# mkofler96/DeepSDF

Measured on AMD Instinct MI355X. Metric: SDF point-samples/sec per training step (8x512 decoder, 16384 pts), higher is better.
Workload: dtype f32; 1 GPU; configs[1]: 64 synthetic sphere-SDF scenes, latent_dim=256, 8x512 decoder + layer-4 skip, weight-norm, dropout 0.2, 16384 pts/step (64 scenes x 256 samples), fp32; headline_config=True, parallelism=dp1

## Files before the change

deepsdf_amd/csrc/dsdf_api.hip:

```cpp
#include "../../include/dsdf.h"

#include <hip/hip_runtime.h>
#include <math.h>
#include <stdarg.h>
#include <stdio.h>
#include <string.h>

#include <stdlib.h>

#include <algorithm>
#include <atomic>
#ifdef DSDF_LAB
#include <vector>
#endif

#include "dwstream.hpp"
#include "sample.hpp"
#include "fused.hpp"
#include "fused_bf16x8.hpp"
#include "gemm.hpp"
#include "kernels.hpp"
#include "mcubes.hpp"
#include "meshsdf.hpp"
#include "msgrid.hpp"
// ... 1052 lines not shown
  R.dw_busy = want_dw ? ((R.dw_items + 3) / 4 < R.cus ? (R.dw_items + 3) / 4 : R.cus) : 0;
  static const bool no_ride = [] { const char* e = getenv("DSDF_NO_RIDE"); return e && e[0] == '1'; }();
  R.rides = segmode && want_dw && R.cus - R.dw_busy >= 8 && c.P.nwg <= R.cus && !no_ride && !c.net->gemm_split && phase <= 1 &&
            R.dw_items > 0;
  if (R.rides) {
    q.lat.nslice = 1; R.lat_slices = 1;
    q.lat_bx = 0;
    R.lat_n = (c.net->latent_size + 15) / 16;
    q.rr_n = q.rr_bx;
    q.dw_n = (q.dw.out[0] + SDW_ROWS_RIDE - 1) / SDW_ROWS_RIDE + (ks > 0 ? (q.dw.out[1] + SDW_ROWS_RIDE - 1) / SDW_ROWS_RIDE : 0);
  }
  return R;
}

int launch_dw(const Call& c, const DwSched& DS, const Roles& R, bool segmode, int phase) {
  const int last = c.net->n_layers - 1;
  DwArgs d;
  memset(&d, 0, sizeof(d));
  d.n_layers = last; d.n_full = DS.n_full; d.n_narrow = DS.n_narrow; d.N = (int)c.n;
  double fl = 0;
  for (int l = 0; l < last; ++l) {
    DwLayer& y = d.ly[l];
    y.dp = c.at<float>(c.P.dpl_off[l]); y.ld_dp = c.P.ld_dp;
    y.act = c.at<float>(c.P.in_off[l]); y.ld_act = c.P.ld_in[l];
    y.slabs = c.at<float>(c.P.dwslab_off[l]); y.slab = DS.slab[l];
    y.M = c.net->out_dim[l]; y.Nc = dw_cols(c.net, l, segmode); y.ldc = c.P.ld_in[l];
    y.tiles_m = DS.tiles_m[l]; y.tiles_n = DS.tiles_n[l]; y.last_nj = DS.last_nj[l]; y.nfull_n = DS.nfull_n[l];
    y.nsplit = DS.nsplit[l]; y.kchunk = DS.kchunk[l]; y.full0 = DS.full0[l]; y.narrow0 = DS.narrow0[l];
    if (in_phase(c.P, phase, l)) fl += 2.0 * (double)c.n * y.M * c.net->in_dim[l];
  }
#ifdef DSDF_LAB
  static LabStamps stamps{"DSDF_LAB_DWDBG", 1024 * 4 * 8 * 8, true, nullptr};
  LabScope lab(stamps, c.st);
  d.dbg = stamps.dev;
#endif
  ProfScope ps(DSDF_PROF_DW_STREAM, fl, c.st);
  const DwKernel kernel = KERNELS[c.path.family].dw;
  if (R.rides) {
    hipLaunchKernelGGL(kernel, dim3(R.cus), dim3(256), 0, c.st, d, R.q, R.lat_n, R.dw_busy);
  } else {
    PostBwdArgs none;
    memset(&none, 0, sizeof(none));
    const int grid = R.dw_busy < 1 ? 1 : R.dw_busy;
    hipLaunchKernelGGL(kernel, dim3(grid), dim3(256), 0, c.st, d, none, 0, grid);
  }
  LAUNCH_OK("dw_stream_kernel");
  return 0;
}

int fin_table(const Call& c, const DwSched& DS, const GradSink& to, bool segmode, int phase, FinAll* fa) {
  const int last = c.net->n_layers - 1, ks = skip_layer(c.net);
  memset(fa, 0, sizeof(*fa));
  int rows = 0;
  for (int l = last; l >= 0; --l) {
    if (!in_phase(c.P, phase, l)) continue;
    FinSrc src;
    if (l == last) src = FinSrc{c.at<float>(c.P.part2_off), LAST_GROUPS, c.P.ld_part, c.P.ld_part, c.at<float>(c.P.partdb_off), c.P.nwg, 1};
    else if (l == last - 1)
      src = FinSrc{c.at<float>(c.P.dwslab_off[l]), DS.nsplit[l], DS.slab[l], c.P.ld_in[l], c.at<float>(c.P.part2_off) + c.P.ld_in[last], LAST_GROUPS, c.P.ld_part};
    else src = FinSrc{c.at<float>(c.P.dwslab_off[l]), DS.nsplit[l], DS.slab[l], c.P.ld_in[l], c.at<float>(c.P.cs_off[l]), c.P.nwg, c.P.ldcs};
    FinArgs& f = fa->f[fa->n];
    f = fin_args(c, l, src, to);
    if (segmode && (l == 0 || l == ks)) {
      f.hoist = 1; f.lat0 = l == 0 ? 0 : c.net->out_dim[l - 1]; f.hW = c.net->latent_size + c.net->geom_dim; f.ldh = c.P.ldh;
      f.hs = c.at<float>(c.P.hs_off) + (l == 0 ? 0 : c.P.hstride);
    }
    fa->row0[fa->n] = rows;
    rows += fin_blocks(f.out, f.in);
    ++fa->n;
  }
  fa->row0[fa->n] = rows;
  return rows;
}

int run_backward_fused(const Call& c, const GradSink& to, int ncols_dz, bool* used_dzB, bool want_dw, const FusedBwdHead& head,
                       const SegBwd* sb, const FusedFwdArgs* fwd, int phase) {
  const DwSched& DS = phase == 0 ? c.P.dw : c.P.dwph[phase - 1];
  const bool segmode = sb != nullptr;
  FusedBwdArgs a = dx_chain_args(c, ncols_dz, want_dw, head, sb, used_dzB);
  if (phase <= 1) TRY(launch_dx_chain(c, a, fwd));
  const Roles R = plan_roles(c, DS, want_dw, sb, phase);
  if (!segmode && phase <= 1 && want_dw) {
    hipLaunchKernelGGL(reduce_rows_kernel, dim3(R.rr_bx, LAST_GROUPS), dim3(256), 0, c.st, R.rr);
    LAUNCH_OK("reduce_rows_kernel");
  }
  if (segmode && sb->scatter != nullptr) { sb->scatter->nslice = R.lat_slices; sb->scatter->slice_stride = (long long)sb->R * c.net->latent_size; }
  if (segmode && !R.rides && phase <= 1) {
    hipLaunchKernelGGL(post_bwd_kernel, dim3((unsigned)(R.q.rr_n + R.q.dw_n + R.lat_n)), dim3(256), 0, c.st, R.q, R.lat_n);
    LAUNCH_OK("post_bwd_kernel");
  }
  if (!want_dw) return 0;
  if (R.dw_items > 0) TRY(launch_dw(c, DS, R, segmode, phase));
  FinAll fa;
  const int rows = fin_table(c, DS, to, segmode, phase, &fa);
  if (rows == 0) return 0;
  if (segmode && sb->scatter != nullptr && phase <= 1) {
    hipLaunchKernelGGL(finalize_scatter_kernel, dim3(rows + sb->R), dim3(256), 0, c.st, fa, *sb->scatter, rows);
    LAUNCH_OK("finalize_scatter_kernel");
    *sb->scatter_done = true;
  } else {
    hipLaunchKernelGGL(finalize_all_kernel, dim3(rows), dim3(256), 0, c.st, fa);
    LAUNCH_OK("finalize_all_kernel");
  }
  return 0;
}

FusedBwdHead make_head(const Call& c, int mode) {
  const int last = c.net->n_layers - 1;
  FusedBwdHead h;
  memset(&h, 0, sizeof(h));
  h.mode = mode;
  h.a_last = c.at<float>(c.P.in_off[last]); h.ld_a = c.P.ld_in[last]; h.in_last = c.net->in_dim[last];
  h.w_last = c.packed + c.pk.w_off[last]; h.b_last = c.params + c.L.bias_off[last]; h.use_tanh = c.net->use_tanh;
// ... 1867 lines not shown
```

deepsdf_amd/csrc/dwstream.hpp:

```cpp
#pragma once
#include "common.hpp"
#include "fused.hpp"
#include "kernels.hpp"

namespace dsdf {

struct DwLayer {
  const float* dp; int ld_dp;
  const float* act; int ld_act;
  float* slabs; long long slab;
  int M, Nc, ldc;
  int tiles_m, tiles_n;
  int last_nj;
  int nfull_n;
  int nsplit, kchunk;
  int full0, narrow0;
};
struct DwArgs { int n_layers, n_full, n_narrow, N; DwLayer ly[DSDF_MAX_LAYERS];
                unsigned long long* dbg; };

#ifndef DW_RING_STEPS
#define DW_RING_STEPS 16
#endif
constexpr int DW_RING = DW_RING_STEPS;

template <int NJ> struct DwVec;
template <> struct DwVec<1> { typedef float type; };
template <> struct DwVec<2> { typedef float2 type; };
template <> struct DwVec<3> { typedef float3 type; };
template <> struct DwVec<4> { typedef float4 type; };

template <int NJ>
__device__ __forceinline__ void dw_item(const DwLayer& L, int N, int split, int m0, int n0, int kbeg, int kend, int fr, int fh) {
  typedef typename DwVec<NJ>::type bvec;
  const int nsteps = (kend - kbeg) >> 1;
  const float* bq = L.act + (size_t)(kbeg + fh) * L.ld_act + n0 + NJ * fr;
  const size_t bstep = (size_t)2 * L.ld_act;
  typedef uint32_t u32x4 __attribute__((ext_vector_type(4)));
  const size_t rows_left = (size_t)(N - kbeg);
  const int ra_bytes = (int)min(rows_left * L.ld_dp * 4, (size_t)0x7FFFFFFF), rb_bytes = (int)min(rows_left * L.ld_act * 4, (size_t)0x7FFFFFFF);
  const __amdgpu_buffer_rsrc_t ra = __builtin_amdgcn_make_buffer_rsrc((void*)(L.dp + (size_t)kbeg * L.ld_dp), 0, ra_bytes, 0x00020000);
  const __amdgpu_buffer_rsrc_t rb = __builtin_amdgcn_make_buffer_rsrc((void*)(L.act + (size_t)kbeg * L.ld_act), 0, rb_bytes, 0x00020000);
  const int voa = (fh * L.ld_dp + m0 + 4 * fr) * 4, vob = (fh * L.ld_act + n0 + NJ * fr) * 4;
  const int astepb = 8 * L.ld_dp, bstepb = 8 * L.ld_act;
  auto lda = [&](int q) -> float4 {
    const u32x4 r = __builtin_amdgcn_raw_buffer_load_b128(ra, voa, q * astepb, 0);
    return make_float4(__uint_as_float(r.x), __uint_as_float(r.y), __uint_as_float(r.z), __uint_as_float(r.w));
  };

  f32x16 acc[4][NJ];
#pragma unroll
  for (int i = 0; i < 4; ++i)
#pragma unroll
    for (int j = 0; j < NJ; ++j)
#pragma unroll
      for (int r = 0; r < 16; ++r) acc[i][j][r] = 0.f;

  float4 rga[DW_RING];
  bvec rgb[DW_RING];
  auto ldb = [&](const float* q) -> bvec {
    if constexpr (NJ == 3) { bvec v; v.x = q[0]; v.y = q[1]; v.z = q[2]; return v; }
    else return *reinterpret_cast<const bvec*>(q);
  };
  auto ldbq = [&](int q) -> bvec {
    if constexpr (NJ == 4) {
      const u32x4 r = __builtin_amdgcn_raw_buffer_load_b128(rb, vob, q * bstepb, 0);
      return make_float4(__uint_as_float(r.x), __uint_as_float(r.y), __uint_as_float(r.z), __uint_as_float(r.w));
    } else return ldb(bq + (size_t)q * bstep);
  };
  auto mma = [&](const float4& a, const bvec& b) {
    const float av[4] = {a.x, a.y, a.z, a.w};
    float bv[NJ];
    if constexpr (NJ == 1) bv[0] = b;
    else { bv[0] = b.x; bv[1] = b.y; if constexpr (NJ > 2) bv[2] = b.z; if constexpr (NJ > 3) bv[3] = b.w; }
#pragma unroll
    for (int i = 0; i < 4; ++i)
#pragma unroll
      for (int j = 0; j < NJ; ++j) acc[i][j] = __builtin_amdgcn_mfma_f32_32x32x2f32(av[i], bv[j], acc[i][j], 0, 0, 0);
  };
  if (nsteps > 0) {
    const int last = nsteps - 1;
#pragma unroll
    for (int q = 0; q < DW_RING - 1; ++q) {
      rga[q] = lda(min(q, last));
      rgb[q] = ldbq(min(q, last));
    }
    int s = 0;
    for (; s + DW_RING <= nsteps; s += DW_RING) {
#pragma unroll
      for (int q = 0; q < DW_RING; ++q) {
        const int nxt = min(s + q + DW_RING - 1, last);
        rga[(q + DW_RING - 1) % DW_RING] = lda(nxt);
        rgb[(q + DW_RING - 1) % DW_RING] = ldbq(nxt);
        mma(rga[q], rgb[q]);
        if constexpr (NJ == 4) {
          __builtin_amdgcn_sched_group_barrier(0x020, 1, 0);
          __builtin_amdgcn_sched_group_barrier(0x008, 8, 0);
          __builtin_amdgcn_sched_group_barrier(0x020, 1, 0);
          __builtin_amdgcn_sched_group_barrier(0x008, 8, 0);
        }
      }
    }
#pragma unroll
    for (int q = 0; q < DW_RING - 1; ++q)
      if (s + q < nsteps) mma(rga[q], rgb[q]);
  }
  if ((kend - kbeg) & 1) {
    const int k = kend - 1;
    float4 a = make_float4(0.f, 0.f, 0.f, 0.f);
    bvec b;
    if constexpr (NJ == 1) b = 0.f; else { b.x = 0.f; b.y = 0.f; if constexpr (NJ > 2) b.z = 0.f; if constexpr (NJ > 3) b.w = 0.f; }
    if (fh == 0) {
      a = *reinterpret_cast<const float4*>(L.dp + (size_t)k * L.ld_dp + m0 + 4 * fr);
      b = ldb(L.act + (size_t)k * L.ld_act + n0 + NJ * fr);
    }
    mma(a, b);
  }

  float* slab = L.slabs + (size_t)split * L.slab;
  __amdgpu_buffer_rsrc_t rs = __builtin_amdgcn_make_buffer_rsrc((void*)slab, 0, L.M * L.ldc * 4, 0x00020000);
  const int n = n0 + NJ * fr;
#pragma unroll
  for (int i = 0; i < 4; ++i)
#pragma unroll
    for (int r = 0; r < 16; ++r) {
      const int m = m0 + 4 * (crow(r) + 4 * fh) + i;
      if constexpr (NJ == 4) {
        typedef uint32_t u32x4 __attribute__((ext_vector_type(4)));
        const uint32_t voff = n < L.ldc ? (uint32_t)((m * L.ldc + n) * 4) : 0x7FFFFFFFu;
        u32x4 v = {__float_as_uint(acc[i][0][r]), __float_as_uint(acc[i][1][r]), __float_as_uint(acc[i][2][r]),
                   __float_as_uint(acc[i][3][r])};
        __builtin_amdgcn_raw_buffer_store_b128(v, rs, voff, 0, 0);
      } else {
#pragma unroll
        for (int j = 0; j < NJ; ++j) {
          const uint32_t voff = n + j < L.ldc ? (uint32_t)((m * L.ldc + n + j) * 4) : 0x7FFFFFFFu;
          __builtin_amdgcn_raw_buffer_store_b32(__float_as_uint(acc[i][j][r]), rs, voff, 0, 0);
        }
      }
    }
}

constexpr int DWS_RING = 4;
constexpr int DWS_SLOT = 2 * 16 * 256;

__device__ __forceinline__ Split3 split8v(const float (&x)[8]) {
  typedef uint32_t u32x4 __attribute__((ext_vector_type(4)));
  uint32_t hw[4], mw[4], lw[4];
#pragma unroll
  for (int pr = 0; pr < 4; ++pr) cut_pair(x[2 * pr], x[2 * pr + 1], hw[pr], mw[pr], lw[pr]);
  Split3 s;
  s.h = __builtin_bit_cast(bf16x8, (u32x4){hw[0], hw[1], hw[2], hw[3]});
  s.m = __builtin_bit_cast(bf16x8, (u32x4){mw[0], mw[1], mw[2], mw[3]});
  s.l = __builtin_bit_cast(bf16x8, (u32x4){lw[0], lw[1], lw[2], lw[3]});
  return s;
}

typedef float dw_f32x4 __attribute__((ext_vector_type(4)));
template <int J> __device__ __forceinline__ float dw_comp(const dw_f32x4& v) { return J == 0 ? v.x : (J == 1 ? v.y : (J == 2 ? v.z : v.w)); }
struct DwRaw { dw_f32x4 v[8]; };

__device__ __forceinline__ void dw_block_split(const DwLayer& L, int split, int tmb, int tnb, int kbeg, int kend, int w, int lane, float* ring) {
  typedef uint32_t u32x4 __attribute__((ext_vector_type(4)));
  typedef __attribute__((address_space(3))) void* lds_ptr;
  typedef __attribute__((address_space(3))) const float* lds_cf;
  const int fr = lane & 31, fh = lane >> 5;
  const int npts = kend - kbeg, nsteps = (npts + 15) >> 4;
  const __amdgpu_buffer_rsrc_t ra = __builtin_amdgcn_make_buffer_rsrc((void*)(L.dp + (size_t)kbeg * L.ld_dp), 0, npts * L.ld_dp * 4, 0x00020000);
  const __amdgpu_buffer_rsrc_t rb = __builtin_amdgcn_make_buffer_rsrc((void*)(L.act + (size_t)kbeg * L.ld_act), 0, npts * L.ld_act * 4, 0x00020000);
  const int pva = (tmb * 128 + 4 * lane) * 4, pvb = (tnb * 128 + 4 * lane) * 4;
  auto issue = [&](int st) __attribute__((always_inline)) {
    float* slot = ring + (st % DWS_RING) * DWS_SLOT;
#pragma unroll
    for (int rr = 0; rr < 4; ++rr) {
      const int row = 4 * w + rr, pt = 16 * st + row;
      __builtin_amdgcn_raw_ptr_buffer_load_lds(ra, (lds_ptr)(slot + row * 256), 16, pt * L.ld_dp * 4 + pva, 0, 0, 0);
      __builtin_amdgcn_raw_ptr_buffer_load_lds(rb, (lds_ptr)(slot + 4096 + row * 256), 16, pt * L.ld_act * 4 + pvb, 0, 0, 0);
    }
  };
  int lda4 = L.ld_dp * 4, ldb4 = L.ld_act * 4;
  asm volatile("" : "+s"(lda4), "+s"(ldb4));
  auto issue_row = [&](int st, int rr) __attribute__((always_inline)) {
    float* slot = ring + (st % DWS_RING) * DWS_SLOT;
    int row = 4 * w + rr;
    asm volatile("" : "+s"(row));
    const int pt = 16 * st + row;
    __builtin_amdgcn_raw_ptr_buffer_load_lds(ra, (lds_ptr)(slot + row * 256), 16, pt * lda4 + pva, 0, 0, 0);
    __builtin_amdgcn_raw_ptr_buffer_load_lds(rb, (lds_ptr)(slot + 4096 + row * 256), 16, pt * ldb4 + pvb, 0, 0, 0);
  };
  const int ca = (w >> 1) * 128 + 4 * fr, cb = 4096 + (w & 1) * 128 + 4 * fr;
#define DW_READ_RAW(ST, A, B, WAITSTR)                                                                                              \
  {                                                                                                                                 \
    const float* slot_ = ring + ((ST) % DWS_RING) * DWS_SLOT;                                                                       \
// ... 123 lines not shown
#undef DW_SBSEL
#undef DW_SA_OF
#undef DW_WAIT_LGKM
#undef DW_READ_RAW
  __builtin_amdgcn_s_waitcnt(0x0F70);
  __syncthreads();
  const int m0 = (tmb + (w >> 1)) * 128, n0 = (tnb + (w & 1)) * 128;
  float* slab = L.slabs + (size_t)split * L.slab;
  __amdgpu_buffer_rsrc_t rs = __builtin_amdgcn_make_buffer_rsrc((void*)slab, 0, L.M * L.ldc * 4, 0x00020000);
  const int n = n0 + 4 * fr;
#pragma unroll
  for (int i = 0; i < 4; ++i)
#pragma unroll
    for (int rg = 0; rg < 16; ++rg) {
      const int m = m0 + 4 * (crow(rg) + 4 * fh) + i;
      const uint32_t voff = n < L.ldc ? (uint32_t)((m * L.ldc + n) * 4) : 0x7FFFFFFFu;
      u32x4 v = {__float_as_uint(acc[i][0][rg]), __float_as_uint(acc[i][1][rg]), __float_as_uint(acc[i][2][rg]),
                 __float_as_uint(acc[i][3][rg])};
      __builtin_amdgcn_raw_buffer_store_b128(v, rs, voff, 0, 0);
    }
}

template <bool SPLIT>
__device__ __forceinline__ void dw_stream_body(const DwArgs& p, const PostBwdArgs& post, const int post_lat_n, const int busy_wg,
                                               float* ring) {
  const int lane = threadIdx.x & 63, w = __builtin_amdgcn_readfirstlane(threadIdx.x >> 6);
  const int fr = lane & 31, fh = lane >> 5;
  const int lwg = xcd_remap(blockIdx.x, gridDim.x);
#ifdef DSDF_LAB
  unsigned long long* const dbgw = p.dbg ? p.dbg + (size_t)(lwg * 4 + w) * 8 : nullptr;
  if (dbgw && lane == 0) { dbgw[0] = __builtin_amdgcn_s_memrealtime(); dbgw[2] = lwg >= busy_wg; }
#endif
  if (lwg >= busy_wg) {
    if constexpr (SPLIT) return;
    const int total = post.rr_n + post.dw_n + post_lat_n;
#ifdef DSDF_LAB
    unsigned long long tk[3] = {0, 0, 0};
#endif
    for (int i = lwg - busy_wg; i < total; i += (int)gridDim.x - busy_wg) {
      __syncthreads();
#ifdef DSDF_LAB
      const unsigned long long t0 = __builtin_amdgcn_s_memrealtime();
#endif
      post_bwd_role_ride(post, i, post_lat_n, ring);
#ifdef DSDF_LAB
      tk[i < post.rr_n ? 0 : (i < post.rr_n + post.dw_n ? 1 : 2)] += __builtin_amdgcn_s_memrealtime() - t0;
#endif
    }
#ifdef DSDF_LAB
    if (dbgw && lane == 0) { dbgw[1] = __builtin_amdgcn_s_memrealtime(); dbgw[3] = tk[0]; dbgw[4] = tk[1]; dbgw[5] = tk[2]; }
#endif
    return;
  }
  const int nwaves = busy_wg * 4;
  const int wave = lwg * 4 + w;
  for (int item = wave; item - w < p.n_full; item += nwaves) {
    if constexpr (SPLIT) {
      const int item0 = item - w;
      int l0 = 0;
      while (l0 + 1 < p.n_layers && item0 >= p.ly[l0 + 1].full0) ++l0;
      const DwLayer& L0 = p.ly[l0];
      const int tf0 = L0.tiles_m * L0.nfull_n, local0 = item0 - L0.full0;
      const bool block = item0 + 3 < p.n_full && (l0 + 1 >= p.n_layers || item0 + 3 < p.ly[l0 + 1].full0) && !(L0.tiles_m & 1) &&
                         !(L0.nfull_n & 1) && !(local0 & 3) && !(tf0 & 3);
      if (block) {
        const int split = local0 / tf0, b = (local0 - split * tf0) >> 2, nbn = L0.nfull_n >> 1;
        const int kbeg = split * L0.kchunk;
        dw_block_split(L0, split, 2 * (b / nbn), 2 * (b % nbn), kbeg, min(p.N, kbeg + L0.kchunk), w, lane, ring);
        continue;
      }
    }
    if (item >= p.n_full) continue;
    int l = 0;
    while (l + 1 < p.n_layers && item >= p.ly[l + 1].full0) ++l;
    const DwLayer& L = p.ly[l];
    const int tf = L.tiles_m * L.nfull_n;
    const int local = item - L.full0;
    const int split = local / tf, tile = local - split * tf;
    const int kbeg = split * L.kchunk;
    int tm = tile / L.nfull_n, tn = tile - tm * L.nfull_n;
    if (!(L.tiles_m & 1) && !(L.nfull_n & 1)) {
      const int nbn = L.nfull_n >> 1, b = tile >> 2, i = tile & 3;
      tm = 2 * (b / nbn) + (i >> 1);
      tn = 2 * (b % nbn) + (i & 1);
    }
    dw_item<4>(L, p.N, split, tm * 128, tn * 128, kbeg, min(p.N, kbeg + L.kchunk), fr, fh);
  }
  if (p.n_narrow > 0) {
    const int used = p.n_full % nwaves;
    const int spare = used == 0 ? nwaves : nwaves - used;
    const int first = used == 0 ? 0 : used;
    if (wave >= first) {
      for (int item = wave - first; item < p.n_narrow; item += spare) {
        int l = 0;
        while (l + 1 < p.n_layers && item >= p.ly[l + 1].narrow0) ++l;
        const DwLayer& L = p.ly[l];
        const int local = item - L.narrow0;
        const int split = local / L.tiles_m, tm = local - split * L.tiles_m;
        const int kbeg = split * L.kchunk, kend = min(p.N, kbeg + L.kchunk);
        const int m0 = tm * 128, n0 = (L.tiles_n - 1) * 128;
        switch (L.last_nj) {
          case 1: dw_item<1>(L, p.N, split, m0, n0, kbeg, kend, fr, fh); break;
          case 2: dw_item<2>(L, p.N, split, m0, n0, kbeg, kend, fr, fh); break;
          default: dw_item<3>(L, p.N, split, m0, n0, kbeg, kend, fr, fh); break;
        }
      }
    }
  }
#ifdef DSDF_LAB
  if (dbgw && lane == 0) dbgw[1] = __builtin_amdgcn_s_memrealtime();
#endif
}

__global__ __launch_bounds__(256, 1) void dw_stream_kernel(const DwArgs p, const PostBwdArgs post, const int post_lat_n,
                                                           const int busy_wg) {
  __shared__ __attribute__((aligned(16))) float role_lds[ROLE_LDS_FLOATS];
  dw_stream_body<false>(p, post, post_lat_n, busy_wg, role_lds);
}
__global__ __launch_bounds__(256, 1) void dw_stream_split_kernel(const DwArgs p, const PostBwdArgs post, const int post_lat_n,
                                                                 const int busy_wg) {
  __shared__ __attribute__((aligned(16))) float ring[DWS_RING * DWS_SLOT];
  static_assert(DWS_RING * DWS_SLOT >= ROLE_LDS_FLOATS, "the roles' scratch must fit the ring");
  dw_stream_body<true>(p, post, post_lat_n, busy_wg, ring);
}

}
```

deepsdf_amd/csrc/kernels.hpp:

```cpp
#pragma once
#include "common.hpp"

namespace dsdf {

constexpr int FSEG_MAXW = 512;

__global__ void latent_renorm_kernel(float* __restrict__ table, int L, const int64_t* __restrict__ seg_scene,
                                     int R, float max_norm, float* __restrict__ dlat, long long nzero) {
  if (dlat != nullptr)
    for (long long i = ((long long)blockIdx.x * blockDim.x + threadIdx.x) * 4; i < nzero; i += (long long)gridDim.x * blockDim.x * 4) {
      if (i + 3 < nzero) *reinterpret_cast<float4*>(dlat + i) = make_float4(0.f, 0.f, 0.f, 0.f);
      else for (long long q = i; q < nzero; ++q) dlat[q] = 0.f;
    }
  const int r = blockIdx.x * (blockDim.x >> 6) + (threadIdx.x >> 6);
  const int lane = threadIdx.x & 63;
  if (r >= R || max_norm <= 0.f) return;
  const int64_t j = seg_scene[r];
  int dup = 0;
  for (int q = lane; q < r; q += 64) dup |= (seg_scene[q] == j);
  if (__any(dup)) return;
  float* row = table + (size_t)j * L;
  float ss = 0.f;
  for (int c = lane; c < L; c += 64) { const float v = row[c]; ss += v * v; }
  ss = wave_sum(ss);
// ... 607 lines not shown
  }
  if (p.g) {
    dot = block_sum_256(dot, red);
    ss = block_sum_256(ss, red);
    const float nrm = sqrtf(ss);
    const float gi = p.g[i];
    const float dgi = dot / nrm;
    const float a = gi / nrm, b = gi * dgi / (nrm * nrm);
    float ssn = 0.f;
#pragma unroll
    for (int k = 0; k < MAXC; ++k) {
      const int c = tid + 256 * k;
      if (c < p.in) {
        const size_t o = (size_t)i * p.in + c;
        const float d = a * dwr[k] - b * p.v[o];
        if (p.adam) { const float vn = adam_elem(p.pv[o], d, p.mv[o], p.sv[o], p); ssn += vn * vn; }
        else p.dv[o] = p.accumulate ? p.dv[o] + d : d;
      }
    }
    if (p.adam) {
      ssn = block_sum_256(ssn, red);
      if (tid == 0) {
        const float gn = adam_elem(p.pg[i], dgi, p.mg[i], p.sg[i], p);
        p.scale_out[i] = gn / sqrtf(ssn);
      }
    } else if (tid == 0) p.dg[i] = p.accumulate ? p.dg[i] + dgi : dgi;
  } else {
#pragma unroll
    for (int k = 0; k < MAXC; ++k) {
      const int c = tid + 256 * k;
      if (c < p.in) {
        const size_t o = (size_t)i * p.in + c;
        if (p.adam) adam_elem(p.pv[o], dwr[k], p.mv[o], p.sv[o], p);
        else p.dv[o] = p.accumulate ? p.dv[o] + dwr[k] : dwr[k];
      }
    }
    if (p.adam && tid == 0) p.scale_out[i] = 1.f;
  }
  float s = 0.f;
  for (int q = tid; q < p.npart; q += 256) s += p.colsum[(size_t)q * p.ldcs + i];
  s = block_sum_256(s, red);
  if (tid == 0) {
    if (p.adam) adam_elem(p.pb[i], s, p.mb[i], p.sb[i], p);
    else p.db[i] = p.accumulate ? p.db[i] + s : s;
  }
}

__global__ __launch_bounds__(256) void finalize_layer_kernel(const FinArgs p) {
  __shared__ float red[4];
  finalize_row(p, blockIdx.x, red);
}

constexpr int FW_MAXK = 8;
template <int FW_KU>
__device__ __forceinline__ void finalize_row_wave(const FinArgs& p, const int i) {
  const int lane = threadIdx.x & 63;
  float vv[FW_KU], mo[FW_KU], so[FW_KU], dwr[FW_KU];
  const size_t ro = (size_t)i * p.in;
  const float* mp = p.adam ? p.mv : p.v;
  const float* sp_ = p.adam ? p.sv : p.v;
#pragma unroll
  for (int k = 0; k < FW_KU; ++k) {
    const int c = lane + 64 * k, cc = min(c, p.in - 1);
    const float a0 = p.v[ro + cc], a1 = mp[ro + cc], a2 = sp_[ro + cc];
    const bool ok = c < p.in;
    vv[k] = ok ? a0 : 0.f; mo[k] = ok ? a1 : 0.f; so[k] = ok ? a2 : 0.f;
  }
  float bs = 0.f;
  for (int q0 = lane; q0 < p.npart; q0 += 256) {
    float t[4];
#pragma unroll
    for (int u = 0; u < 4; ++u) t[u] = p.colsum[(size_t)min(q0 + 64 * u, p.npart - 1) * p.ldcs + i];
#pragma unroll
    for (int u = 0; u < 4; ++u) bs += q0 + 64 * u < p.npart ? t[u] : 0.f;
  }
#pragma unroll
  for (int k = 0; k < FW_KU; ++k) dwr[k] = 0.f;
  constexpr int FW_SB = 32 / FW_KU;
  for (int sp = 0; sp < p.nsplit; sp += FW_SB) {
    float t[FW_SB][FW_KU];
#pragma unroll
    for (int u = 0; u < FW_SB; ++u)
#pragma unroll
      for (int k = 0; k < FW_KU; ++k)
        t[u][k] = p.slabs[(size_t)min(sp + u, p.nsplit - 1) * p.slab + (size_t)i * p.ldc + min(lane + 64 * k, p.in - 1)];
#pragma unroll
    for (int u = 0; u < FW_SB; ++u)
#pragma unroll
      for (int k = 0; k < FW_KU; ++k) {
        const int c = lane + 64 * k;
        dwr[k] += (sp + u < p.nsplit && c < p.in && (!p.hoist || c < p.lat0)) ? t[u][k] : 0.f;
      }
  }
  if (p.hoist) {
#pragma unroll
    for (int k = 0; k < FW_KU; ++k) {
      const int c = lane + 64 * k - p.lat0;
      if (c >= 0 && c < p.hW) dwr[k] += p.hs[(size_t)i * p.ldh + c];
    }
  }
  bs = wave_sum(bs);
  if (p.g) {
    float dot = 0.f, ss = 0.f;
#pragma unroll
    for (int k = 0; k < FW_KU; ++k) { dot += dwr[k] * vv[k]; ss += vv[k] * vv[k]; }
    dot = wave_sum(dot);
    ss = wave_sum(ss);
    const float nrm = sqrtf(ss);
    const float gi = p.g[i];
    const float dgi = dot / nrm;
    const float a = gi / nrm, b = gi * dgi / (nrm * nrm);
    float ssn = 0.f;
#pragma unroll
    for (int k = 0; k < FW_KU; ++k) {
      const int c = lane + 64 * k;
      if (c < p.in) {
        const float d = a * dwr[k] - b * vv[k];
        if (p.adam) {
          float pn = vv[k];
          const float vn = adam_elem(pn, d, mo[k], so[k], p);
          p.pv[ro + c] = vn; p.mv[ro + c] = mo[k]; p.sv[ro + c] = so[k];
          ssn += vn * vn;
        } else p.dv[ro + c] = p.accumulate ? p.dv[ro + c] + d : d;
      }
    }
    if (p.adam) {
      ssn = wave_sum(ssn);
      if (lane == 0) {
        const float gn = adam_elem(p.pg[i], dgi, p.mg[i], p.sg[i], p);
        p.scale_out[i] = gn / sqrtf(ssn);
      }
    } else if (lane == 0) p.dg[i] = p.accumulate ? p.dg[i] + dgi : dgi;
  } else {
#pragma unroll
    for (int k = 0; k < FW_KU; ++k) {
      const int c = lane + 64 * k;
      if (c < p.in) {
        if (p.adam) {
          float pn = vv[k];
          adam_elem(pn, dwr[k], mo[k], so[k], p);
          p.pv[ro + c] = pn; p.mv[ro + c] = mo[k]; p.sv[ro + c] = so[k];
        } else p.dv[ro + c] = p.accumulate ? p.dv[ro + c] + dwr[k] : dwr[k];
      }
    }
    if (p.adam && lane == 0) p.scale_out[i] = 1.f;
  }
  if (lane == 0) {
    if (p.adam) adam_elem(p.pb[i], bs, p.mb[i], p.sb[i], p);
    else p.db[i] = p.accumulate ? p.db[i] + bs : bs;
  }
}

struct FinAll { int n; int row0[DSDF_MAX_LAYERS + 1]; FinArgs f[DSDF_MAX_LAYERS]; };
__host__ __device__ inline int fin_blocks(int out, int in) { return in <= 64 * FW_MAXK ? (out + 3) / 4 : out; }
__device__ __forceinline__ void finalize_block(const FinAll& p, const int b, float* red) {
  int l = 0;
  while (l + 1 < p.n && b >= p.row0[l + 1]) ++l;
  const FinArgs& f = p.f[l];
  if (f.in <= 64 * FW_MAXK) {
    const int i = (b - p.row0[l]) * 4 + (int)(threadIdx.x >> 6);
    if (i < f.out) {
      const int ku = (f.in + 63) >> 6;
      if (ku <= 1) finalize_row_wave<1>(f, i);
      else if (ku == 2) finalize_row_wave<2>(f, i);
      else if (ku <= 4) finalize_row_wave<4>(f, i);
      else finalize_row_wave<8>(f, i);
    }
  } else finalize_row(f, b - p.row0[l], red);
}
__global__ __launch_bounds__(256) void finalize_all_kernel(const FinAll p) {
  __shared__ float red[4];
  finalize_block(p, (int)blockIdx.x, red);
}

struct SegArgs {
  const float* dzA; const float* dzB; int ldz;
  const int64_t* seg_scene; const int64_t* seg_offset; int R; int L;
  const float* table;
  float* segpart;
  float* segnorm;
  int nslice; long long slice_stride;
};
__global__ __launch_bounds__(256) void seg_reduce_kernel(const SegArgs p) {
  __shared__ float red[4][64];
  const int r = blockIdx.x, c0 = blockIdx.y * 64;
  const int tid = threadIdx.x, cx = tid & 63, ry = tid >> 6;
  const int64_t sbeg = p.seg_offset[r], send = p.seg_offset[r + 1];
  const int64_t per = (send - sbeg + gridDim.z - 1) / gridDim.z;
  const int64_t beg = min(sbeg + (int64_t)blockIdx.z * per, send), end = min(beg + per, send);
  const int col = c0 + cx, cc = min(col, p.L - 1);
  float s = 0.f;
  for (int64_t n = beg + ry; n < end; n += 32) {
    float t[8];
#pragma unroll
    for (int u = 0; u < 8; ++u) {
      const int64_t m = min(n + 4 * u, end - 1);
      t[u] = p.dzA[(size_t)m * p.ldz + cc];
      if (p.dzB) t[u] += p.dzB[(size_t)m * p.ldz + cc];
    }
#pragma unroll
    for (int u = 0; u < 8; ++u) s += n + 4 * u < end ? t[u] : 0.f;
  }
  red[ry][cx] = s;
  __syncthreads();
  if (ry == 0 && col < p.L)
    p.segpart[(size_t)blockIdx.z * p.slice_stride + (size_t)r * p.L + col] = (red[0][cx] + red[1][cx]) + (red[2][cx] + red[3][cx]);
  if (blockIdx.y == 0 && blockIdx.z == 0 && tid < 64) {
    const float* row = p.table + (size_t)p.seg_scene[r] * p.L;
    float ss = 0.f;
    for (int c = tid; c < p.L; c += 64) { const float v = row[c]; ss += v * v; }
    ss = wave_sum(ss);
    if (tid == 0) p.segnorm[r] = sqrtf(ss);
  }
}

struct SegLatArgs {
  const float* cs0; int ldcs; int out0; const float* W0; int ldw0;
  const float* csk; int outk; const float* Wk; int ldwk; int koff;
  int wg_per_seg; int R; int L;
  const int64_t* seg_scene; const float* table;
  const float* zr;
  float* segpart; float* segnorm;
  int nslice, nchunk; long long slice_stride;
// ... 323 lines not shown

struct ScatterArgs {
  const float* segpart; const float* segnorm; const int64_t* seg_scene; const int64_t* seg_offset; int R; int L;
  float* table; float* dlat; float creg;
  int nslice; long long slice_stride;
  const float* zr;
  const float* part_loss; int n_part; float loss_scale; float* loss_out; int accumulate;
};
__device__ __forceinline__ void seg_scatter_body(const ScatterArgs& p, int r) {
  __shared__ float red[4];
  __shared__ int dup;
  const int tid = threadIdx.x;
  if (r == 0) {
    float s = 0.f;
    if (p.creg != 0.f)
      for (int q = tid; q < p.R; q += 256) s += p.creg * (float)(p.seg_offset[q + 1] - p.seg_offset[q]) * p.segnorm[q];
    s = block_sum_256(s, red);
    float d = 0.f;
    for (int q = tid; q < p.n_part; q += 256) d += p.part_loss[q];
    d = block_sum_256(d, red);
    if (tid == 0) {
      const float v = d * p.loss_scale + s;
      *p.loss_out = p.accumulate ? *p.loss_out + v : v;
    }
  }
  const int64_t j = p.seg_scene[r];
  if (tid == 0) dup = 0;
  __syncthreads();
  int d = 0;
  for (int q = tid; q < r; q += 256) d |= (p.seg_scene[q] == j);
  if (d) dup = 1;
  __syncthreads();
  if (dup) return;
  for (int c = tid; c < p.L; c += 256) {
    const float z = p.zr != nullptr ? p.zr[(size_t)r * p.L + c] : p.table[(size_t)j * p.L + c];
    float acc = 0.f;
    for (int q = r; q < p.R; ++q) {
      if (q != r && p.seg_scene[q] != j) continue;
      float v = p.segpart[(size_t)q * p.L + c];
      for (int sl = 1; sl < p.nslice; ++sl) v += p.segpart[(size_t)sl * p.slice_stride + (size_t)q * p.L + c];
      if (p.creg != 0.f) {
        const float nrm = p.segnorm[q];
        if (nrm > 0.f) v += p.creg * (float)(p.seg_offset[q + 1] - p.seg_offset[q]) * z / nrm;
      }
      acc += v;
    }
    p.dlat[(size_t)j * p.L + c] += acc;
    if (p.zr != nullptr) p.table[(size_t)j * p.L + c] = z;
  }
}

__global__ __launch_bounds__(256) void seg_scatter_kernel(const ScatterArgs p) { seg_scatter_body(p, blockIdx.x); }

__global__ __launch_bounds__(256) void finalize_scatter_kernel(const FinAll p, const ScatterArgs sc, const int rows) {
  if ((int)blockIdx.x < sc.R) { seg_scatter_body(sc, (int)blockIdx.x); return; }
  __shared__ float red[4];
  finalize_block(p, (int)blockIdx.x - sc.R, red);
}

__global__ __launch_bounds__(256) void adam_kernel(float* __restrict__ p, const float* __restrict__ g,
                                                   float* __restrict__ m, float* __restrict__ v, long long n,
                                                   float one_minus_b1, float b2, float one_minus_b2, float step_size,
                                                   float bc2_sqrt, float eps, const float* gscale) {
  const float gs = gscale ? *gscale : 1.f;
  for (long long i = (long long)blockIdx.x * 256 + threadIdx.x; i < n; i += (long long)gridDim.x * 256) {
    const float gi = g[i] * gs;
    const float mi = fmaf(one_minus_b1, gi - m[i], m[i]);
    const float vi = b2 * v[i] + one_minus_b2 * gi * gi;
    m[i] = mi; v[i] = vi;
    p[i] = p[i] - step_size * (mi / (sqrtf(vi) / bc2_sqrt + eps));
  }
}

__global__ __launch_bounds__(256) void adam_sched_kernel(float* __restrict__ p, const float* __restrict__ g, float* __restrict__ m,
                                                         float* __restrict__ v, long long n, const float* __restrict__ sched,
                                                         long long n_steps, const long long* __restrict__ counter, float one_minus_b1,
                                                         float b2, float one_minus_b2, float eps, float l2) {
  long long it = *counter;
  if (it >= n_steps) it = n_steps - 1;
  const float step_size = sched[2 * it], bc2_sqrt = sched[2 * it + 1];
  for (long long i = (long long)blockIdx.x * 256 + threadIdx.x; i < n; i += (long long)gridDim.x * 256) {
    const float gi = fmaf(l2, p[i], g[i]);
    const float mi = fmaf(one_minus_b1, gi - m[i], m[i]);
    const float vi = b2 * v[i] + one_minus_b2 * gi * gi;
    m[i] = mi; v[i] = vi;
    p[i] = p[i] - step_size * (mi / (sqrtf(vi) / bc2_sqrt + eps));
  }
}
__global__ void counter_inc_kernel(long long* counter) { *counter += 1; }

struct AdamRowsLayer { long long v_off, g_off, b_off; int out, in, row0; };
struct AdamRowsArgs {
  int nl, total_rows;
  float* p; const float* g; float* m; float* s;
  float* scale;
  float omb1, b2, omb2, step_size, bc2_sqrt, eps; const float* gscale;
  AdamRowsLayer ly[DSDF_MAX_LAYERS];
};
__global__ __launch_bounds__(256) void adam_rows_kernel(const AdamRowsArgs a) {
  const int gr = blockIdx.x * 4 + (threadIdx.x >> 6), lane = threadIdx.x & 63;
  if (gr >= a.total_rows) return;
  int l = 0;
  while (l + 1 < a.nl && gr >= a.ly[l + 1].row0) ++l;
  const AdamRowsLayer& L = a.ly[l];
  const int row = gr - L.row0;
  const float gs = a.gscale ? *a.gscale : 1.f;
  auto upd = [&](long long i) -> float {
// ... 164 lines not shown
```

Measured before the change: 13.33 million point-samples/s.

## Pair neighbouring waves to reduce dW split-K partials through LDS before storing slabs

```diff
diff --git a/deepsdf_amd/csrc/dsdf_api.hip b/deepsdf_amd/csrc/dsdf_api.hip
--- a/deepsdf_amd/csrc/dsdf_api.hip
+++ b/deepsdf_amd/csrc/dsdf_api.hip
@@ -1128,13 +1128,15 @@
   const int last = c.net->n_layers - 1, ks = skip_layer(c.net);
   memset(fa, 0, sizeof(*fa));
   int rows = 0;
+  const int group = KERNELS[c.path.family].dw == dw_stream_kernel ? DW_GROUP : 1;
   for (int l = last; l >= 0; --l) {
     if (!in_phase(c.P, phase, l)) continue;
+    const int live = l == last ? 0 : dw_live_slabs(group, DS.nsplit[l], DS.tiles_m[l], DS.nfull_n[l], DS.last_nj[l], DS.full0[l]);
     FinSrc src;
     if (l == last) src = FinSrc{c.at<float>(c.P.part2_off), LAST_GROUPS, c.P.ld_part, c.P.ld_part, c.at<float>(c.P.partdb_off), c.P.nwg, 1};
     else if (l == last - 1)
-      src = FinSrc{c.at<float>(c.P.dwslab_off[l]), DS.nsplit[l], DS.slab[l], c.P.ld_in[l], c.at<float>(c.P.part2_off) + c.P.ld_in[last], LAST_GROUPS, c.P.ld_part};
-    else src = FinSrc{c.at<float>(c.P.dwslab_off[l]), DS.nsplit[l], DS.slab[l], c.P.ld_in[l], c.at<float>(c.P.cs_off[l]), c.P.nwg, c.P.ldcs};
+      src = FinSrc{c.at<float>(c.P.dwslab_off[l]), live, DS.slab[l], c.P.ld_in[l], c.at<float>(c.P.part2_off) + c.P.ld_in[last], LAST_GROUPS, c.P.ld_part};
+    else src = FinSrc{c.at<float>(c.P.dwslab_off[l]), live, DS.slab[l], c.P.ld_in[l], c.at<float>(c.P.cs_off[l]), c.P.nwg, c.P.ldcs};
     FinArgs& f = fa->f[fa->n];
     f = fin_args(c, l, src, to);
     if (segmode && (l == 0 || l == ks)) {
diff --git a/deepsdf_amd/csrc/dwstream.hpp b/deepsdf_amd/csrc/dwstream.hpp
--- a/deepsdf_amd/csrc/dwstream.hpp
+++ b/deepsdf_amd/csrc/dwstream.hpp
@@ -24,14 +24,31 @@
 #endif
 constexpr int DW_RING = DW_RING_STEPS;
 
+#ifndef DW_GROUP_SIZE
+#define DW_GROUP_SIZE 2
+#endif
+constexpr int DW_GROUP = DW_GROUP_SIZE;
+static_assert(DW_GROUP == 1 || DW_GROUP == 2, "a group is one wave or a pair of neighbouring waves");
+constexpr int DW_XCH_FLOATS = 2 * 64 * 256;
+__host__ __device__ inline int dw_grouped_splits(int group, int nsplit, int tiles_m, int nfull_n, int last_nj, int full0) {
+  const int tf = tiles_m * nfull_n;
+  if (group == 1 || last_nj != 4 || tf == 0 || (full0 & 3) || tf % (4 / group)) return 0;
+  return nsplit / group * group;
+}
+__host__ __device__ inline int dw_live_slabs(int group, int nsplit, int tiles_m, int nfull_n, int last_nj, int full0) {
+  const int gs = dw_grouped_splits(group, nsplit, tiles_m, nfull_n, last_nj, full0);
+  return gs / group + (nsplit - gs);
+}
+
 template <int NJ> struct DwVec;
 template <> struct DwVec<1> { typedef float type; };
 template <> struct DwVec<2> { typedef float2 type; };
 template <> struct DwVec<3> { typedef float3 type; };
 template <> struct DwVec<4> { typedef float4 type; };
 
-template <int NJ>
-__device__ __forceinline__ void dw_item(const DwLayer& L, int N, int split, int m0, int n0, int kbeg, int kend, int fr, int fh) {
+template <int NJ, int G = 1>
+__device__ __forceinline__ void dw_item(const DwLayer& L, int N, int slabi, int m0, int n0, int kbeg, int kend, int fr, int fh,
+                                        int member = -1, int w = 0, float* xch = nullptr) {
   typedef typename DwVec<NJ>::type bvec;
   const int nsteps = (kend - kbeg) >> 1;
   const float* bq = L.act + (size_t)(kbeg + fh) * L.ld_act + n0 + NJ * fr;
@@ -117,11 +134,58 @@
     mma(a, b);
   }
 
-  float* slab = L.slabs + (size_t)split * L.slab;
+  [[maybe_unused]] auto pin_row = [&](int i) { asm volatile("" : "+a"(acc[i][0]), "+a"(acc[i][1]), "+a"(acc[i][2]), "+a"(acc[i][3])); };
+  typedef float f32x4 __attribute__((ext_vector_type(4)));
+  [[maybe_unused]] const f32x4* partner = nullptr;
+  if constexpr (NJ == 4 && G > 1) {
+    if (member >= 0) {
+      f32x4* region = reinterpret_cast<f32x4*>(xch + (w >> 1) * (DW_XCH_FLOATS / 2)) + (fr + 32 * fh);
+      if (member == 1) {
+#pragma unroll
+        for (int i = 0; i < 4; ++i) {
+          pin_row(i);
+#pragma unroll
+          for (int j = 0; j < 4; ++j)
+#pragma unroll
+            for (int q = 0; q < 4; ++q)
+              region[((i * 4 + j) * 4 + q) * 64] = (f32x4){acc[i][j][4 * q], acc[i][j][4 * q + 1], acc[i][j][4 * q + 2], acc[i][j][4 * q + 3]};
+        }
+      }
+      __syncthreads();
+      if (member == 1) return;
+      partner = region;
+    }
+  }
+  float* slab = L.slabs + (size_t)slabi * L.slab;
   __amdgpu_buffer_rsrc_t rs = __builtin_amdgcn_make_buffer_rsrc((void*)slab, 0, L.M * L.ldc * 4, 0x00020000);
   const int n = n0 + NJ * fr;
-#pragma unroll
-  for (int i = 0; i < 4; ++i)
+  if constexpr (NJ == 4 && G > 1) {
+    if (partner) {
+      typedef uint32_t u32x4 __attribute__((ext_vector_type(4)));
+#pragma unroll
+      for (int i = 0; i < 4; ++i) {
+        pin_row(i);
+        f32x4 t[4][4];
+#pragma unroll
+        for (int j = 0; j < 4; ++j)
+#pragma unroll
+          for (int q = 0; q < 4; ++q) t[j][q] = partner[((i * 4 + j) * 4 + q) * 64];
+#pragma unroll
+        for (int r = 0; r < 16; ++r) {
+          const int m = m0 + 4 * (crow(r) + 4 * fh) + i;
+          const uint32_t voff = n < L.ldc ? (uint32_t)((m * L.ldc + n) * 4) : 0x7FFFFFFFu;
+          u32x4 v = {__float_as_uint(acc[i][0][r] + t[0][r >> 2][r & 3]), __float_as_uint(acc[i][1][r] + t[1][r >> 2][r & 3]),
+                     __float_as_uint(acc[i][2][r] + t[2][r >> 2][r & 3]), __float_as_uint(acc[i][3][r] + t[3][r >> 2][r & 3])};
+          __builtin_amdgcn_raw_buffer_store_b128(v, rs, voff, 0, 0);
+        }
+        __builtin_amdgcn_sched_barrier(0);
+      }
+      return;
+    }
+  }
+#pragma unroll
+  for (int i = 0; i < 4; ++i) {
+    if constexpr (NJ == 4 && G > 1) pin_row(i);
 #pragma unroll
     for (int r = 0; r < 16; ++r) {
       const int m = m0 + 4 * (crow(r) + 4 * fh) + i;
@@ -139,6 +203,7 @@
         }
       }
     }
+  }
 }
 
 constexpr int DWS_RING = 4;
@@ -368,6 +433,7 @@
 #endif
     return;
   }
+  constexpr int G = SPLIT ? 1 : DW_GROUP;
   const int nwaves = busy_wg * 4;
   const int wave = lwg * 4 + w;
   for (int item = wave; item - w < p.n_full; item += nwaves) {
@@ -392,7 +458,15 @@
     const DwLayer& L = p.ly[l];
     const int tf = L.tiles_m * L.nfull_n;
     const int local = item - L.full0;
-    const int split = local / tf, tile = local - split * tf;
+    int split = local / tf, tile = local - split * tf, slabi = split, member = -1;
+    if constexpr (G > 1) {
+      const int gs = dw_grouped_splits(G, L.nsplit, L.tiles_m, L.nfull_n, L.last_nj, L.full0);
+      if (local < gs * tf) {
+        const int gg = local / (G * tf), r = local - gg * G * tf;
+        member = w % G;
+        split = gg * G + member; tile = (r >> 2) * (4 / G) + w / G; slabi = gg;
+      } else slabi = gs / G + (split - gs);
+    }
     const int kbeg = split * L.kchunk;
     int tm = tile / L.nfull_n, tn = tile - tm * L.nfull_n;
     if (!(L.tiles_m & 1) && !(L.nfull_n & 1)) {
@@ -400,7 +474,7 @@
       tm = 2 * (b / nbn) + (i >> 1);
       tn = 2 * (b % nbn) + (i & 1);
     }
-    dw_item<4>(L, p.N, split, tm * 128, tn * 128, kbeg, min(p.N, kbeg + L.kchunk), fr, fh);
+    dw_item<4, G>(L, p.N, slabi, tm * 128, tn * 128, kbeg, min(p.N, kbeg + L.kchunk), fr, fh, member, w, ring);
   }
   if (p.n_narrow > 0) {
     const int used = p.n_full % nwaves;
@@ -430,8 +504,9 @@
 
 __global__ __launch_bounds__(256, 1) void dw_stream_kernel(const DwArgs p, const PostBwdArgs post, const int post_lat_n,
                                                            const int busy_wg) {
-  __shared__ __attribute__((aligned(16))) float role_lds[ROLE_LDS_FLOATS];
-  dw_stream_body<false>(p, post, post_lat_n, busy_wg, role_lds);
+  constexpr int LDS_FLOATS = DW_GROUP > 1 && DW_XCH_FLOATS > ROLE_LDS_FLOATS ? DW_XCH_FLOATS : ROLE_LDS_FLOATS;
+  __shared__ __attribute__((aligned(16))) float lds[LDS_FLOATS];
+  dw_stream_body<false>(p, post, post_lat_n, busy_wg, lds);
 }
 __global__ __launch_bounds__(256, 1) void dw_stream_split_kernel(const DwArgs p, const PostBwdArgs post, const int post_lat_n,
                                                                  const int busy_wg) {
```

Result: no change. 13.39 million point-samples/s (median of 6 runs) (+0.5%).

## Restructure per-row wave finalize to batch slab loads and interleave late parameter loads

Applied to the files above, without the earlier changes.

```diff
diff --git a/deepsdf_amd/csrc/kernels.hpp b/deepsdf_amd/csrc/kernels.hpp
--- a/deepsdf_amd/csrc/kernels.hpp
+++ b/deepsdf_amd/csrc/kernels.hpp
@@ -683,52 +683,113 @@
 }
 
 constexpr int FW_MAXK = 8;
+__device__ __forceinline__ float ld_lane_off(const float* base, unsigned byte_off) {
+  return *reinterpret_cast<const float*>(reinterpret_cast<const char*>(base) + byte_off);
+}
+__device__ __forceinline__ float fw_scalar(float rs, int q) { return __int_as_float(__builtin_amdgcn_readlane(__float_as_int(rs), q)); }
+template <int FW_KU> struct FwBatch { static constexpr int SB = 80 / FW_KU; };
 template <int FW_KU>
-__device__ __forceinline__ void finalize_row_wave(const FinArgs& p, const int i) {
+__device__ __forceinline__ void fw_late_loads(const FinArgs& p, const int i, const int lane, const unsigned (&co)[FW_KU], float (&vv)[FW_KU],
+                                              float (&mo)[FW_KU], float (&so)[FW_KU], float (&hv)[FW_KU]) {
+  const size_t ro = (size_t)i * p.in;
+  const float* vp = p.v + ro;
+  const float* mp = (p.adam ? p.mv : p.v) + ro;
+  const float* sp_ = (p.adam ? p.sv : p.v) + ro;
+#pragma unroll
+  for (int k = 0; k < FW_KU; ++k) {
+    const float a0 = ld_lane_off(vp, co[k]), a1 = ld_lane_off(mp, co[k]), a2 = ld_lane_off(sp_, co[k]);
+    const bool ok = lane + 64 * k < p.in;
+    vv[k] = ok ? a0 : 0.f; mo[k] = ok ? a1 : 0.f; so[k] = ok ? a2 : 0.f;
+  }
+#pragma unroll
+  for (int k = 0; k < FW_KU; ++k) hv[k] = 0.f;
+  if (p.hoist) {
+    const float* hr = p.hs + (size_t)i * p.ldh;
+#pragma unroll
+    for (int k = 0; k < FW_KU; ++k) hv[k] = ld_lane_off(hr, 4u * (unsigned)min(max(lane + 64 * k - p.lat0, 0), p.hW - 1));
+  }
+}
+template <int FW_KU, int NB, bool FIRST>
+__device__ __forceinline__ void fw_slab_batch(const FinArgs& p, const int i, const int lane, const int sp, unsigned (&co)[FW_KU],
+                                              float (&dwr)[FW_KU], float (&vv)[FW_KU], float (&mo)[FW_KU], float (&so)[FW_KU],
+                                              float (&hv)[FW_KU]) {
+  const float* rowp = p.nsplit > 0 ? p.slabs + (size_t)i * p.ldc : p.v + (size_t)i * p.in;
+  float t[FW_KU][NB];
+#pragma unroll
+  for (int k = 0; k < FW_KU; ++k)
+#pragma unroll
+    for (int u = 0; u < NB; ++u) t[k][u] = ld_lane_off(rowp + (size_t)max(min(sp + u, p.nsplit - 1), 0) * p.slab, co[k]);
+  constexpr int KH = !FIRST ? FW_KU : FW_KU / 2;
+  constexpr int UH = FIRST && FW_KU == 1 ? NB / 2 : 0;
+#pragma unroll
+  for (int k = 0; k < FW_KU; ++k) {
+    if (FIRST && k == KH) {
+#pragma unroll
+      for (int q = 0; q < FW_KU; ++q) asm volatile("" : "+v"(dwr[q < KH ? q : 0]), "+v"(co[q]));
+      fw_late_loads<FW_KU>(p, i, lane, co, vv, mo, so, hv);
+    }
+    const int c = lane + 64 * k;
+#pragma unroll
+    for (int u = 0; u < NB; ++u) {
+      if (FIRST && FW_KU == 1 && u == UH) {
+        asm volatile("" : "+v"(dwr[0]), "+v"(co[0]));
+        fw_late_loads<FW_KU>(p, i, lane, co, vv, mo, so, hv);
+      }
+      dwr[k] += (sp + u < p.nsplit && c < p.in && (!p.hoist || c < p.lat0)) ? t[k][u] : 0.f;
+    }
+  }
+}
+template <int FW_KU>
+__device__ __forceinline__ void finalize_row_wave(const FinArgs& p, const int row) {
   const int lane = threadIdx.x & 63;
-  float vv[FW_KU], mo[FW_KU], so[FW_KU], dwr[FW_KU];
+  const int i = __builtin_amdgcn_readfirstlane(row);
+  float vv[FW_KU], mo[FW_KU], so[FW_KU], dwr[FW_KU], hv[FW_KU];
+  unsigned co[FW_KU];
   const size_t ro = (size_t)i * p.in;
-  const float* mp = p.adam ? p.mv : p.v;
-  const float* sp_ = p.adam ? p.sv : p.v;
-#pragma unroll
-  for (int k = 0; k < FW_KU; ++k) {
-    const int c = lane + 64 * k, cc = min(c, p.in - 1);
-    const float a0 = p.v[ro + cc], a1 = mp[ro + cc], a2 = sp_[ro + cc];
-    const bool ok = c < p.in;
-    vv[k] = ok ? a0 : 0.f; mo[k] = ok ? a1 : 0.f; so[k] = ok ? a2 : 0.f;
-  }
-  float bs = 0.f;
-  for (int q0 = lane; q0 < p.npart; q0 += 256) {
-    float t[4];
-#pragma unroll
-    for (int u = 0; u < 4; ++u) t[u] = p.colsum[(size_t)min(q0 + 64 * u, p.npart - 1) * p.ldcs + i];
-#pragma unroll
-    for (int u = 0; u < 4; ++u) bs += q0 + 64 * u < p.npart ? t[u] : 0.f;
+#pragma unroll
+  for (int k = 0; k < FW_KU; ++k) co[k] = 4u * (unsigned)min(lane + 64 * k, p.in - 1);
+  const float* sq = p.v + ro;
+  if (p.g && lane == 0) sq = p.g + i;
+  if (p.adam) {
+    if (lane == 1) sq = p.pb + i;
+    if (lane == 2) sq = p.mb + i;
+    if (lane == 3) sq = p.sb + i;
+    if (p.g) {
+      if (lane == 4) sq = p.pg + i;
+      if (lane == 5) sq = p.mg + i;
+      if (lane == 6) sq = p.sg + i;
+    }
+  }
+  const float rs = *sq;
+  float tb[4] = {0.f, 0.f, 0.f, 0.f};
+  if (p.npart > 0) {
+    const float* cs = p.colsum + i;
+#pragma unroll
+    for (int u = 0; u < 4; ++u) tb[u] = cs[(size_t)min(lane + 64 * u, p.npart - 1) * p.ldcs];
   }
 #pragma unroll
   for (int k = 0; k < FW_KU; ++k) dwr[k] = 0.f;
-  constexpr int FW_SB = 32 / FW_KU;
-  for (int sp = 0; sp < p.nsplit; sp += FW_SB) {
-    float t[FW_SB][FW_KU];
-#pragma unroll
-    for (int u = 0; u < FW_SB; ++u)
-#pragma unroll
-      for (int k = 0; k < FW_KU; ++k)
-        t[u][k] = p.slabs[(size_t)min(sp + u, p.nsplit - 1) * p.slab + (size_t)i * p.ldc + min(lane + 64 * k, p.in - 1)];
-#pragma unroll
-    for (int u = 0; u < FW_SB; ++u)
-#pragma unroll
-      for (int k = 0; k < FW_KU; ++k) {
-        const int c = lane + 64 * k;
-        dwr[k] += (sp + u < p.nsplit && c < p.in && (!p.hoist || c < p.lat0)) ? t[u][k] : 0.f;
-      }
+  {
+    constexpr int FW_SB = FwBatch<FW_KU>::SB;
+    fw_slab_batch<FW_KU, FW_SB, true>(p, i, lane, 0, co, dwr, vv, mo, so, hv);
+    for (int sp = FW_SB; sp < p.nsplit; sp += FW_SB) fw_slab_batch<FW_KU, FW_SB, false>(p, i, lane, sp, co, dwr, vv, mo, so, hv);
   }
   if (p.hoist) {
 #pragma unroll
     for (int k = 0; k < FW_KU; ++k) {
       const int c = lane + 64 * k - p.lat0;
-      if (c >= 0 && c < p.hW) dwr[k] += p.hs[(size_t)i * p.ldh + c];
-    }
+      if (c >= 0 && c < p.hW) dwr[k] += hv[k];
+    }
+  }
+  float bs = 0.f;
+#pragma unroll
+  for (int u = 0; u < 4; ++u) bs += lane + 64 * u < p.npart ? tb[u] : 0.f;
+  for (int q0 = lane + 256; q0 < p.npart; q0 += 256) {
+    float t[4];
+#pragma unroll
+    for (int u = 0; u < 4; ++u) t[u] = p.colsum[(size_t)min(q0 + 64 * u, p.npart - 1) * p.ldcs + i];
+#pragma unroll
+    for (int u = 0; u < 4; ++u) bs += q0 + 64 * u < p.npart ? t[u] : 0.f;
   }
   bs = wave_sum(bs);
   if (p.g) {
@@ -738,7 +799,7 @@
     dot = wave_sum(dot);
     ss = wave_sum(ss);
     const float nrm = sqrtf(ss);
-    const float gi = p.g[i];
+    const float gi = fw_scalar(rs, 0);
     const float dgi = dot / nrm;
     const float a = gi / nrm, b = gi * dgi / (nrm * nrm);
     float ssn = 0.f;
@@ -758,7 +819,9 @@
     if (p.adam) {
       ssn = wave_sum(ssn);
       if (lane == 0) {
-        const float gn = adam_elem(p.pg[i], dgi, p.mg[i], p.sg[i], p);
+        float pn = fw_scalar(rs, 4), mn = fw_scalar(rs, 5), sn = fw_scalar(rs, 6);
+        const float gn = adam_elem(pn, dgi, mn, sn, p);
+        p.pg[i] = gn; p.mg[i] = mn; p.sg[i] = sn;
         p.scale_out[i] = gn / sqrtf(ssn);
       }
     } else if (lane == 0) p.dg[i] = p.accumulate ? p.dg[i] + dgi : dgi;
@@ -777,8 +840,11 @@
     if (p.adam && lane == 0) p.scale_out[i] = 1.f;
   }
   if (lane == 0) {
-    if (p.adam) adam_elem(p.pb[i], bs, p.mb[i], p.sb[i], p);
-    else p.db[i] = p.accumulate ? p.db[i] + bs : bs;
+    if (p.adam) {
+      float pn = fw_scalar(rs, 1), mn = fw_scalar(rs, 2), sn = fw_scalar(rs, 3);
+      adam_elem(pn, bs, mn, sn, p);
+      p.pb[i] = pn; p.mb[i] = mn; p.sb[i] = sn;
+    } else p.db[i] = p.accumulate ? p.db[i] + bs : bs;
   }
 }
 
@@ -799,7 +865,7 @@
     }
   } else finalize_row(f, b - p.row0[l], red);
 }
-__global__ __launch_bounds__(256) void finalize_all_kernel(const FinAll p) {
+__global__ __launch_bounds__(256) __attribute__((amdgpu_waves_per_eu(4))) void finalize_all_kernel(const FinAll p) {
   __shared__ float red[4];
   finalize_block(p, (int)blockIdx.x, red);
 }
@@ -1229,7 +1295,7 @@
 
 __global__ __launch_bounds__(256) void seg_scatter_kernel(const ScatterArgs p) { seg_scatter_body(p, blockIdx.x); }
 
-__global__ __launch_bounds__(256) void finalize_scatter_kernel(const FinAll p, const ScatterArgs sc, const int rows) {
+__global__ __launch_bounds__(256) __attribute__((amdgpu_waves_per_eu(4))) void finalize_scatter_kernel(const FinAll p, const ScatterArgs sc, const int rows) {
   if ((int)blockIdx.x < sc.R) { seg_scatter_body(sc, (int)blockIdx.x); return; }
   __shared__ float red[4];
   finalize_block(p, (int)blockIdx.x - sc.R, red);
```

After: 13.27 million point-samples/s before, 13.26 million point-samples/s after. About the same (-0.1%).
